# microsoft/MaskFlownet

Hardware: AMD Instinct MI355X
Metric: image-pairs/s MaskFlownet-S 384x512 fwd hot path (correlation + deformable conv + warp) (higher is better)
Workload: dtype f32

## Files before the change

include/mfn_hip.h:

```cpp
#ifndef MFN_HIP_H
#define MFN_HIP_H

#include <stddef.h>

#ifdef __cplusplus
extern "C" {
#endif

#define MFN_ABI_VERSION 1

#define MFN_OK 0
#define MFN_E_NULL (-1)
#define MFN_E_SHAPE (-2)
#define MFN_E_PARAM (-3)
#define MFN_E_UNSUPPORTED (-4)
#define MFN_E_WORKSPACE (-5)
#define MFN_E_ALIGN (-6)

#define MFN_REQ_NULL 0
#define MFN_REQ_WRITE 1
#define MFN_REQ_ADD 3

int mfn_abi_version(void);
const char *mfn_version_string(void);
// ... 196 lines not shown
int mfn_graph_destroy(void *graph_exec);

int mfn_profile_enable(int on);
int mfn_profile_reset(void);
int mfn_profile_tag(const char *tag);
int mfn_profile_query(const char *name_substr, int *launches, double *total_ms);
int mfn_profile_dump(char *buf, int cap);

#define MFN_ARITH_DEFAULT (-1)
#define MFN_ARITH_FP32 0
#define MFN_ARITH_BF16X3 1
int mfn_set_arithmetic(const char *op, int mode);
int mfn_get_arithmetic(const char *op, int *mode);

int mfn_debug_set_timeline(void *device_buffer);
int mfn_set_tuning(const char *key, int value);
int mfn_get_tuning(const char *key, int *value);

#ifdef __cplusplus
}
#endif
#endif
```

maskflownet_amd/_abi.py:

```python
import ctypes as C
from types import SimpleNamespace

_f = C.c_void_p
_i = C.c_int
_s = C.c_void_p
_pi = C.POINTER(C.c_int)

SIGNATURES = {
    "last_error": (C.c_char_p, []),
    "correlation_out_shape": (_i, [_i] * 7 + [_pi, _pi, _pi]),
    "correlation_fwd": (_i, [_f, _f, _f] + [_i] * 10 + [_s]),
    "correlation_workspace_bytes": (C.c_size_t, [_i] * 10),
    "correlation_fwd_ws": (_i, [_f, _f, _f] + [_i] * 10 + [C.c_void_p, C.c_size_t, _s]),
    "correlation_fwd_act": (_i, [_f, _f, _f] + [_i] * 11 + [C.c_void_p, C.c_size_t, _s]),
    "correlation_fwd_into": (_i, [_f, _f, _f, C.c_longlong] + [_i] * 11 + [C.c_void_p, C.c_size_t, _s]),
    "warp_fwd": (_i, [_f, _f, _f] + [_i] * 5 + [_s]),
    "grid_generator_warp": (_i, [_f, _f, _i, _i, _i, _s]),
    "grid_generator_affine": (_i, [_f, _f, _i, _i, _i, _s]),
    "bilinear_sampler_fwd": (_i, [_f, _f, _f] + [_i] * 6 + [_s]),
    "bilinear_sampler_bwd": (_i, [_f] * 5 + [_i] * 8 + [_s]),
    "grid_generator_warp_bwd": (_i, [_f, _f] + [_i] * 4 + [_s]),
    "deform_conv_out_shape": (_i, [_i] * 10 + [_pi, _pi]),
    "deform_conv_workspace_bytes": (C.c_size_t, [_i] * 15),
    "deform_conv_fwd": (_i, [_f] * 5 + [_i] * 15 + [C.c_void_p, C.c_size_t, _s]),
    "deform_conv_shared_fwd": (_i, [_f, _f, C.c_float, C.c_float, _f, _f, _f] + [_i] * 12 + [C.c_void_p, C.c_size_t, _s]),
    "offsets_from_flow": (_i, [_f, _f, _i, _i, _i, _i, C.c_float, C.c_float, _s]),
    "offsets_from_flow_bwd": (_i, [_f, _f, _i, _i, _i, _i, C.c_float, C.c_float, _i, _s]),
    "deform_conv_shared_bwd_workspace_bytes": (C.c_size_t, [_i] * 12),
    "deform_conv_shared_bwd": (_i, [_f, _f, _f, C.c_float, C.c_float, _f, _f, _f, _f, _f] + [_i] * 16 + [C.c_void_p, C.c_size_t, _s]),
    "debug_set_timeline": (_i, [C.c_void_p]),
    "correlation_bwd": (_i, [_f] * 5 + [_i] * 12 + [_s]),
    "warp_bwd": (_i, [_f] * 5 + [_i] * 7 + [_s]),
    "deform_conv_packed_weight_bytes": (C.c_size_t, [_i] * 15),
    "deform_conv_pack_weights": (_i, [_f] + [_i] * 15 + [C.c_void_p, C.c_size_t, C.POINTER(C.c_ulonglong), _s]),
    "deform_conv_fwd_packed": (_i, [_f, _f, C.c_void_p, C.c_size_t, C.c_ulonglong, _f, _f] + [_i] * 15 + [C.c_void_p, C.c_size_t, _s]),
    "deform_conv_shared_fwd_packed": (_i, [_f, _f, C.c_float, C.c_float, C.c_void_p, C.c_size_t, C.c_ulonglong, _f, _f] + [_i] * 12 + [C.c_void_p, C.c_size_t, _s]),
    "upsample_fwd": (_i, [_f, _f] + [_i] * 5 + [_s]),
    "deform_conv_matching_fwd": (_i, [_f, _f, C.c_float, C.c_float, _f, C.c_void_p, C.c_size_t, C.c_ulonglong, _f, _f, _f, _i, _f]
                                 + [_i] * 12 + [C.c_void_p, C.c_size_t, _s]),
    "deform_conv_bwd_workspace_bytes": (C.c_size_t, [_i] * 15),
    "deform_conv_bwd": (_i, [_f] * 8 + [_i] * 19 + [C.c_void_p, C.c_size_t, _s]),
    "conv2d_out_shape": (_i, [_i] * 13 + [_pi, _pi]),
    "conv2d_workspace_bytes": (C.c_size_t, [_i] * 15),
    "conv2d_packed_weight_bytes": (C.c_size_t, [_i] * 15),
    "conv2d_pack_weights": (_i, [_f] + [_i] * 15 + [C.c_void_p, C.c_size_t, C.POINTER(C.c_ulonglong), _s]),
# ... 75 lines not shown
```

maskflownet_amd/csrc/api_impl.inc:

```

#include <atomic>
#include <math.h>
#include <stdarg.h>
#include <stdio.h>
#include <string.h>

#include "kernels/correlation.h"
#include "kernels/correlation_direct.h"
#include "kernels/correlation_gram.h"
#include "kernels/correlation_gramk.h"
#include "kernels/conv_wgrad.h"
#include "kernels/deform_conv.h"
#include "kernels/deform_conv_mma.h"
#include "kernels/warp.h"
#include "kernels/upsample.h"
#include "kernels/predict.h"
#include "kernels/augment.h"
#include "kernels/loss.h"
#include "kernels/optimizer.h"
#include "kernels/batch.h"
#include "kernels/ingest.h"
#include "kernels/backward.h"
#include "kernels/dc_backward.h"
#include "kernels/conv.h"
// ... 9 lines not shown
  vsnprintf(g_err, sizeof(g_err), fmt, ap);
  va_end(ap);
  return code;
}
static int hipfail(int rc, const char *what) {
  if (rc == 0) return 0;
  snprintf(g_err, sizeof(g_err), "%s: HIP error %d (%s)", what, rc, hipGetErrorString((hipError_t)rc));
  return rc;
}
static inline bool aligned(const void *p, size_t a) { return ((uintptr_t)p % a) == 0; }

Tuning g_tuning;
struct Arith { std::atomic<int> corr{-1}, deform{-1}, conv{-1}; };
static Arith t_arith;
void *g_timeline = nullptr;
struct Settings { Tuning t; int corr, deform, conv; };
static Settings settings_now() { return Settings{g_tuning, t_arith.corr.load(), t_arith.deform.load(), t_arith.conv.load()}; }

static int corr_shape(int H, int W, int md, int kernel, int s1, int s2, int pad, int *tc, int *th, int *tw) {
  if (H <= 0 || W <= 0) return fail(MFN_E_SHAPE, "correlation: H=%d W=%d must be positive", H, W);
  if (md < 0 || kernel < 1 || s1 < 1 || s2 < 1 || pad < 0)
    return fail(MFN_E_PARAM, "correlation: bad parameter (max_displacement=%d kernel_size=%d stride1=%d stride2=%d pad_size=%d)",
                md, kernel, s1, s2, pad);
  if ((kernel % 2) == 0) return fail(MFN_E_PARAM, "correlation: kernel size should be odd number (got %d)", kernel);
  const int Hp = H + 2 * pad, Wp = W + 2 * pad;
  const int border = md + (kernel - 1) / 2;
  const int th_ = (int)ceilf((float)(Hp - border * 2) / (float)s1);
  const int tw_ = (int)ceilf((float)(Wp - border * 2) / (float)s1);
  if (th_ < 1 || tw_ < 1)
    return fail(MFN_E_SHAPE, "correlation: Correlation cannot be done with current settings. Neighborhood and kernel don't fit in blob");
// ... 286 lines not shown
  if (H + 2 * ph < dh * (kh - 1) + 1 || W + 2 * pw < dw * (kw - 1) + 1 || ho < 1 || wo < 1)
    return fail(MFN_E_SHAPE, "deform_conv: kernel size exceed input");
  if (Ho) *Ho = ho;
  if (Wo) *Wo = wo;
  return 0;
}

static bool dc_mfma_ok(const Settings &st, int kh, int kw, int groups, int dg) {
  return (st.t.path_generic & 2) == 0 && kh == 3 && kw == 3 && groups == 1 && dg == 1;
}

struct DcPlan {
  int mt, pt, nw, ksb, mgroups, ncp_pad, cps_per_slice;
  int mma;
  int kw, ring, groups, gps;
  int tile_w, tiles_x, tiles_y, ntiles;
  size_t wt_bytes, partial_bytes, mg_words;
};
#ifndef MFN_DCM_CONFIGS
#define MFN_DCM_CONFIGS(X) X(1, 4, 1) X(2, 3, 4) X(2, 2, 2) X(3, 1, 6) X(1, 1, 8) X(1, 1, 4) X(1, 1, 2) X(1, 1, 1)
#endif
static bool dcm_config_ok(int mt, int pt, int kw) {
#define X(a, b, c) if (mt == a && pt == b && kw == c) return true;
  MFN_DCM_CONFIGS(X)
#undef X
  return false;
}
static DcPlan dc_plan(const Settings &st, int Cin, int Cout, int N, int Ho, int Wo, bool mma_shape) {
  DcPlan pl;
  memset(&pl, 0, sizeof(pl));
  const long P = (long)N * Ho * Wo;
  const int mtiles = (Cout + 31) / 32;
  int mt = 1;
  pl.tile_w = Wo >= 8 ? 8 : 0;
  if (pl.tile_w) {
    pl.tiles_x = (Wo + pl.tile_w - 1) / pl.tile_w;
// ... 9 lines not shown
    pl.groups = Cin / 16;
    pl.ring = 3;
    int cmt = 1, cpt = 1, ckw = pl.groups % 8 == 0 ? 8 : (pl.groups % 4 == 0 ? 4 : (pl.groups % 2 == 0 ? 2 : 1));
    if (mtiles == 1 && tiles >= 1024) { cpt = 4; ckw = 1; }
    else if (mtiles == 2 && tiles >= 384 && pl.groups % 4 == 0) {
      cmt = 2; cpt = 3; ckw = 4;
      if ((tiles + 2) / 3 > 256 && (tiles + 1) / 2 <= 512) { cpt = 2; ckw = 2; }
    }
    else if (mtiles == 3 && pl.groups % 6 == 0) { cmt = 3; ckw = 6; }
    else if (tiles >= 1024) { cpt = 4; ckw = 1; }
    if (st.t.dc_mt > 0 && st.t.dc_pt > 0 && st.t.dc_nw > 0) {
      cmt = st.t.dc_mt; cpt = st.t.dc_pt; ckw = st.t.dc_nw / (cpt > 0 ? cpt : 1);
    }
    if (!dcm_config_ok(cmt, cpt, ckw) || pl.groups % ckw != 0 || cmt > mtiles) { cmt = 1; cpt = 1; ckw = 1; }
    pl.mt = cmt; pl.pt = cpt; pl.kw = ckw; pl.nw = cpt * ckw; pl.ksb = 1;
    pl.mgroups = (mtiles + cmt - 1) / cmt;
    pl.gps = pl.groups / ckw;
    pl.mg_words = (size_t)(pl.groups * 9 + dcm_kc(cmt, ckw)) * (3 * cmt * 256);
    pl.wt_bytes = (pl.mgroups * pl.mg_words * sizeof(float) + 255) / 256 * 256;
    pl.partial_bytes = 0;
    return pl;
  }
  pl.mt = mt;
  pl.mma = 0;
  pl.mgroups = (mtiles + mt - 1) / mt;
  const int ncp = (Cin + 1) / 2;
  int pt = st.t.dc_pt;
  if (!(pt == 1 || pt == 2 || pt == 4)) {
    double best = 1e30;
    pt = 1;
// ... 147 lines not shown
  p.cps_per_slice = pl.cps_per_slice;
  p.ksb = pl.ksb;
  p.mgroups = pl.mgroups;
  p.tile_w = pl.tile_w; p.tiles_x = pl.tiles_x; p.tiles_y = pl.tiles_y; p.ntiles = pl.ntiles;
  p.inv_tpi = pl.tile_w ? 1.0f / (float)(pl.tiles_y * pl.tiles_x) : 0.f;
  p.inv_tiles_x = pl.tile_w ? 1.0f / (float)pl.tiles_x : 0.f;
  p.partial = pl.ksb > 1 ? (float *)partial_base : nullptr;
  rc = -1000;
  if (pl.mma == 2) {
    if (!aligned(p.x, 16) || !aligned(p.out, 16) || !aligned(p.wt, 16))
      return fail(MFN_E_ALIGN, "%s: x, out and the packed weights must be 16-byte aligned for the matrix-core layout these weights were packed in "
                  "(pass the raw weights, or pack under mfn_set_arithmetic(\"deformable_convolution\", MFN_ARITH_FP32))", what);
    p.dcm_groups = pl.groups;
    p.dcm_gps = pl.gps;
    p.xcd = pl.mgroups == 1 || cdiv(pl.ntiles, pl.pt) % 8 == 0;
#define X(a, b, c) else if (pl.mt == a && pl.pt == b && pl.kw == c) rc = dc_mma_launch<a, b, c, 3>(p, s);
    if (false) {}
    MFN_DCM_CONFIGS(X)
#undef X
    if (rc == -1000) return fail(MFN_E_UNSUPPORTED, "%s: no matrix-core kernel for mt=%d pt=%d kw=%d", what, pl.mt, pl.pt, pl.kw);
    return hipfail(rc, what);
  }
  if (pl.nw == 8) rc = dc_lds_launch<1, 1, 8>(p, s, "dc_lds");
  else if (pl.pt == 1) rc = dc_lds_launch<1, 1>(p, s, "dc_lds");
  else if (pl.pt == 2) rc = dc_lds_launch<1, 2>(p, s, "dc_lds");
  else if (pl.pt == 4) rc = dc_lds_launch<1, 4>(p, s, "dc_lds");
  if (rc == -1000) return fail(MFN_E_UNSUPPORTED, "%s: no kernel for mt=%d pt=%d", what, pl.mt, pl.pt);
  if (rc) return hipfail(rc, what);
  if (pl.ksb > 1) {
    DcReduceParams rp{p.partial, p.bias, p.out, (size_t)p.Cout * p.P, pl.ksb, p.Cout, (size_t)p.Ho * p.Wo,
                      p.ep_mask, p.ep_add, p.ep_leaky};
    rc = dc_reduce_launch(rp, s);
// ... 1511 lines not shown
int MFN_API(set_arithmetic)(const char *op, int mode) {
  if (mode < -1 || mode > 1) return fail(MFN_E_PARAM, "set_arithmetic: mode %d is none of MFN_ARITH_DEFAULT / _FP32 / _BF16X3", mode);
  if (op && !strcmp(op, "all")) { t_arith.corr = mode; t_arith.deform = mode; t_arith.conv = mode; return 0; }
  std::atomic<int> *slot = arith_slot(op);
  if (!slot) return fail(MFN_E_PARAM, "set_arithmetic: unknown operator '%s'", op ? op : "(null)");
  *slot = mode;
  return 0;
}
int MFN_API(get_arithmetic)(const char *op, int *mode) {
  std::atomic<int> *slot = arith_slot(op);
  if (!slot || !mode) return fail(MFN_E_PARAM, "get_arithmetic: unknown operator '%s'", op ? op : "(null)");
  *mode = *slot;
  return 0;
}

int MFN_API(set_tuning)(const char *key, int value) {
  int *slot = key ? g_tuning.slot(key) : nullptr;
  if (!slot) return fail(MFN_E_PARAM, "set_tuning: unknown key '%s'", key ? key : "(null)");
  *slot = value;
  return 0;
}
int MFN_API(get_tuning)(const char *key, int *value) {
  int *slot = key ? g_tuning.slot(key) : nullptr;
  if (!slot || !value) return fail(MFN_E_PARAM, "get_tuning: unknown key '%s'", key ? key : "(null)");
  *value = *slot;
  return 0;
}

}
```

maskflownet_amd/csrc/kernels/deform_conv_mma.h:

```cpp
#pragma once
#include "deform_conv.h"
#include "msplit.h"

namespace mfn {

constexpr int DCM_XW_F = 512;
template <bool BIG, int RING> struct DcmWin {
  static constexpr int ROWS = BIG ? 16 : 12, COLS = BIG ? 24 : 20, C4 = COLS / 4, CH = ROWS * COLS;
  static constexpr int CHS = BIG ? CH : 268;
  static constexpr bool IS_BIG = BIG;
  static constexpr int NI = BIG ? 3 : 2, SLOT_F = BIG ? 768 : 512;
  static constexpr int DEPTH = BIG ? (RING * DCM_XW_F) / 768 : RING;
  static_assert(CHS % 4 == 0 && CHS >= CH && CHS + CH <= SLOT_F && CHS + CH <= NI * 256 && DEPTH >= 2, "the pair's window fits its slot and its transfers");
};

template <int RING> struct DcmWinConv {
  static constexpr int ROWS = 6, COLS = 16, C4 = 4, CH = ROWS * COLS, CHS = 104;
  static constexpr int NI = 1, SLOT_F = 256;
  static constexpr int DEPTH = (RING * DCM_XW_F) / SLOT_F;
  static_assert(CHS % 4 == 0 && CHS >= CH && CHS + CH <= SLOT_F && DEPTH >= 2, "the pair's window fits one transfer");
};

constexpr int dcm_kc(int mt, int kw) { return mt * kw == 1 ? 3 : 1; }
constexpr int dcm_nstage(int mt, int pt, int kw, int ring) {
// ... 5 lines not shown
constexpr int dcm_min_waves(int mt, int nw) {
  const int fit = (nw + 3) / 4, want = mt == 1 ? 3 : (mt == 2 ? 2 : 1);
  return fit > want ? fit : want;
}

#ifndef MFN_DCM_ABLATE
#define MFN_DCM_ABLATE 0
#endif
#ifndef MFN_DCM_MSPLIT
#define MFN_DCM_MSPLIT (MT <= 2)
#endif
#ifndef MFN_DCM_MINW
#define MFN_DCM_MINW(mt, nw) dcm_min_waves(mt, nw)
#endif

template <int MT, int PT, int KW, int RING> struct DcmGeom {
  static constexpr int NW = PT * KW, NTH = NW * 64;
  static constexpr int KC = dcm_kc(MT, KW);
  static constexpr int NSTAGE = dcm_nstage(MT, PT, KW, RING);
  static constexpr int STEP_W = 3 * MT * 256;
  static constexpr int WI_TOTAL = KW * KC * 3 * MT;
  static constexpr int NI = (WI_TOTAL + NW - 1) / NW;
  static constexpr int NI_MIN = WI_TOTAL / NW;
  static constexpr int STAGE_W = WI_TOTAL * 256;
  static constexpr int XW_OFF = NSTAGE * STAGE_W;
  static constexpr int T8_OFF = XW_OFF + NW * RING * DCM_XW_F;
  static constexpr int DUMP_OFF = T8_OFF + NW * 512;
  static constexpr int LDS_W = DUMP_OFF + 256;
  static_assert(LDS_W * 4 <= 160 * 1024, "a block's LDS must fit the CU");
  static constexpr int RED_TS = 40, RED_TILE = 32 * RED_TS;
  static constexpr int RED_W = KW > 1 ? PT * KW * MT * RED_TILE : 0;
  static_assert(RED_W <= DUMP_OFF, "every slice's partial tiles fit the block's LDS at once");
  static constexpr int RED_ROWS = 32 * MT, RED_SLAB = RED_ROWS / KW, RED_PASSES = (RED_SLAB + 7) / 8;
  static_assert(RED_ROWS % KW == 0, "the K slices divide the tile's filter rows evenly (every shipped tiling; an uneven split needs a clipped last slab)");
};

template <int KC, int NSTAGE, int RING, int NI, int XW_NI, int REQ = 0> constexpr int dcm_wait_count(int s) {
  int issued = 0, result = 1000;
  int stampW[64] = {}, stampX[80] = {};
  for (int u = 0; u < 45; ++u) {
    const int ss = u % 9, grp = u / 9;
    if (u == 36 + s) {
      int need = -1;
      if (ss % KC == 0 && stampW[u / KC] > need) need = stampW[u / KC];
      if (ss != 7) {
        const int np = ss == 8 ? 8 * (grp + 1) : 8 * grp + ss + 1;
        if (stampX[np] > need) need = stampX[np];
      }
      result = need < 0 ? 1000 : issued - need;
    }
    if (ss % KC == 0) { issued += NI; stampW[u / KC + NSTAGE - 1] = issued; }
    if (ss < 8) { issued += XW_NI; stampX[8 * grp + ss + RING] = issued; }
    if (ss != 7) issued += REQ;
  }
  return result;
}
template <int KC, int NSTAGE, int RING, int NI, int XW_NI, int REQ> constexpr int dcm_landed_count(int s) {
  int issued = 0, last_req = 0, result = 0;
  for (int u = 0; u < 45; ++u) {
    const int ss = u % 9;
    if (ss % KC == 0) issued += NI;
    if (ss < 8) issued += XW_NI;
    if (ss != 7) {
      issued += REQ;
      if (u == 36 + s) result = issued - last_req;
      last_req = issued;
    }
  }
  return result;
}

template <int KC, int NSTAGE, int RING, int NI, int XW_NI> constexpr unsigned dcm_wait_mask(int s) {
  const int v = dcm_wait_count<KC, NSTAGE, RING, NI, XW_NI>(s);
  unsigned m = 0;
  for (int q = 0; q < 9; ++q) {
    if (dcm_wait_count<KC, NSTAGE, RING, NI, XW_NI>(q) != v) continue;
// ... 24 lines not shown
  }
  mfn_bf16x8 h, mm, l;
  mfn_split3x8(x, h, mm, l);
  float *base = p.wt + (size_t)mg * p.mg_words + ((size_t)grp * 9 + s) * (3 * p.MT * 256) + (size_t)(kb * 32 + m) * 4;
  mfn_write_bf16x8(base + (0 * p.MT + ft) * 256, h);
  mfn_write_bf16x8(base + (1 * p.MT + ft) * 256, mm);
  mfn_write_bf16x8(base + (2 * p.MT + ft) * 256, l);
}
inline int dcm_pack_launch(DcmPackParams pp, hipStream_t stream) {
  const size_t total = (size_t)pp.mgroups * pp.ngroups * 9 * pp.MT * 64;
  return launch("dcm_pack_weights", dcm_pack_weights_kernel, dim3((unsigned)((total + 255) / 256)), dim3(256), 0, stream, pp);
}

struct DcmB { mfn_bf16x8 h, m, l; };

template <int MT, int PT, int KW, int RING, bool CONV = false>
__global__ __launch_bounds__(PT * KW * 64, MFN_DCM_MINW(MT, PT * KW)) void dc_mma_kernel(DeformParams p) {
  using G = DcmGeom<MT, PT, KW, RING>;
  constexpr int NW = G::NW, KC = G::KC, NI = G::NI, NIW = G::NI_MIN;
  constexpr int NACC = MT == 1 ? 2 : 1;
  constexpr bool PRIVATE_W = PT == 1;
  static_assert(!PRIVATE_W || G::NI * NW == G::WI_TOTAL, "one pixel tile: the slices' blocks divide evenly over the waves");
  static_assert(9 % KC == 0, "chunk boundaries at fixed steps of a group");
  static_assert(RING >= 3 && RING * DCM_XW_F >= 32 * 40, "the epilogue transposes a tile through the wave's window ring");
  MFN_DYN_SHARED(float, lds);

  const int tid = threadIdx.x;
  const int lane = tid & 63;
  const int wave = MFN_UNIFORM(tid >> 6);
  const int kb = lane >> 5, j = lane & 31;
  const int pt = wave / KW, kw = wave % KW;
  MFN_STAMP(p.timeline, 0);
  const int bx = p.xcd ? (int)mfn_xcd_remap(blockIdx.x, gridDim.x) : (int)blockIdx.x;
  const int tile = bx * PT + pt;
// ... 4 lines not shown
  const size_t xns = p.x_nstride ? p.x_nstride : (size_t)p.Cin * plane;

  const int gps = p.dcm_gps;
  const size_t mg_words = (size_t)(p.dcm_groups * 9 + KC) * G::STEP_W;
  const mfn_rsrc_t wrsrc = mfn_make_rsrc(p.wt + (size_t)mg * mg_words, (unsigned)(mg_words * 4));
  unsigned voffW[NI];
  MFN_UNROLL
  for (int i = 0; i < NI; ++i) {
    const int ii = PRIVATE_W ? wave * (KC * 3 * MT) + i : i * NW + wave;
    const int k = ii / (KC * 3 * MT), rem = ii - k * (KC * 3 * MT);
    voffW[i] = ii < G::WI_TOTAL ? (unsigned)((((size_t)k * gps * 9) * G::STEP_W + (size_t)rem * 256) * 4) + (unsigned)lane * 16u : 0xFFFFFF00u;
  }
  auto issue_w = [&](int ch) {
    float *buf = lds + (ch % G::NSTAGE) * G::STAGE_W;
    const unsigned soff = ch * KC < gps * 9 ? (unsigned)((size_t)ch * KC * G::STEP_W * 4) : 0x7FFFFF00u;
    if (MFN_DCM_ABLATE & 32) return;
    MFN_UNROLL
    for (int i = 0; i < NI; ++i) {
      const int ii = PRIVATE_W ? wave * (KC * 3 * MT) + i : i * NW + wave;
      if (ii < G::WI_TOTAL) mfn_dma16_so(wrsrc, buf + ii * 256, voffW[i], soff);
    }
  };

  MFN_UNROLL
  for (int ch = 0; ch < G::NSTAGE - 1; ++ch) issue_w(ch);

  int n, ty, tx;
  {
    auto divmod = [](int a, int b, float inv_b, int &q, int &r) {
      q = (int)((float)a * inv_b);
      r = a - q * b;
      if (r < 0) { --q; r += b; }
      if (r >= b) { ++q; r -= b; }
    };
    const int tl = min(tile, p.ntiles - 1);
    int rt;
    divmod(tl, p.tiles_y * p.tiles_x, p.inv_tpi, n, rt);
    divmod(rt, p.tiles_x, p.inv_tiles_x, ty, tx);
  }
  const int tile_ho0 = ty * 4, tile_wo0 = tx * 8;
// ... 256 lines not shown
    }
  };
  DcmB B;
  GramSel sel;
  if (MFN_DCM_MSPLIT) sel = gram_make_sel(lane);
  mfn_bf16x8 ah[MT], am[MT], al[MT];
  auto a_read = [&](const float *a) {
    MFN_UNROLL
    for (int ft = 0; ft < MT; ++ft) {
      if (MFN_DCM_ABLATE & 64) { ah[ft] = am[ft] = al[ft] = B.h; continue; }
      al[ft] = mfn_read_bf16x8(a + (2 * MT + ft) * 256);
      ah[ft] = mfn_read_bf16x8(a + (0 * MT + ft) * 256);
      am[ft] = mfn_read_bf16x8(a + (1 * MT + ft) * 256);
    }
  };
  auto mma_issue = [&](const DcmB &b) {
    if (MFN_DCM_ABLATE & 1) {
      MFN_UNROLL
      for (int ft = 0; ft < MT; ++ft) acc[ft][0][0] += mfn_bf16_at(reinterpret_cast<const float *>(&ah[ft]), 0) + mfn_bf16_at(reinterpret_cast<const float *>(&al[ft]), 1) + mfn_bf16_at(reinterpret_cast<const float *>(&am[ft]), 2) + mfn_bf16_at(reinterpret_cast<const float *>(&b.l), 0);
      return;
    }
#define MFN_DCM_(A_, B_, P_)                                                                      \
  MFN_UNROLL                                                                                      \
  for (int ft = 0; ft < MT; ++ft) acc[ft][(P_) % NACC] = MFN_MFMA_32x32x16_BF16(A_[ft], B_, acc[ft][(P_) % NACC]);
    MFN_DCM_(al, b.h, 0)
    MFN_DCM_(ah, b.l, 1)
    MFN_DCM_(am, b.m, 0)
    MFN_DCM_(am, b.h, 1)
    MFN_DCM_(ah, b.m, 0)
    MFN_DCM_(ah, b.h, 1)
// ... 20 lines not shown
        MFN_UNROLL
        for (int ft = 0; ft < MT; ++ft) {
          const float wv = mfn_bf16_at(a + (0 * MT + ft) * 256, t) + mfn_bf16_at(a + (1 * MT + ft) * 256, t) + mfn_bf16_at(a + (2 * MT + ft) * 256, t);
          acc[ft][0] = MFN_MFMA_32x32x2(wv, cvt, acc[ft][0]);
        }
      } else {
        *t8dst = cvt;
      }
    }
  };

  float *xt8 = lds + G::T8_OFF + wave * 512 + lane;
  auto first_operand = [&](auto win_c, auto out_c) {
    using WN = decltype(win_c);
    MFN_WAIT_VM(0);
    float x8[8] = {0.f, 0.f, 0.f, 0.f, 0.f, 0.f, 0.f, 0.f}, c8 = 0.f;
    if (fast) {
      if (decltype(out_c)::value) lanes_request(0, std::integral_constant<int, 1>{});
      cols_gather(0, win_c);
      if (decltype(out_c)::value) {
        lanes_landed(std::integral_constant<int, 1>{}, std::integral_constant<int, 0>{});
        lanes_request(1, std::integral_constant<int, 0>{});
      }
      cols_finish(x8, c8);
    }
    xt8[0] = c8;
    if (MFN_DCM_MSPLIT) gram_msplit8(x8, sel, B.h, B.m, B.l);
    else mfn_split3x8(x8, B.h, B.m, B.l);
    MFN_STAMP2(p.timeline, 4);
  };

  auto run_groups = [&](auto win_c, auto out_c) {
    using WN = decltype(win_c);
    constexpr int CPG = 9 / KC;
    if (decltype(out_c)::value) lanes_setup();
    first_operand(win_c, out_c);
    MFN_NOUNROLL
    for (int g = 0; g < gps; ++g) {
      mfn_static_for<9>([&](auto s_c) {
        constexpr int S = decltype(s_c)::value;
        constexpr bool OUT = decltype(out_c)::value;
        constexpr int NWAIT = dcm_wait_count<KC, G::NSTAGE, WN::DEPTH, NIW, WN::NI, OUT ? 16 : 0>(S);
        if (NWAIT < 1000) MFN_WAIT_VM(NWAIT < 63 ? NWAIT : 63);
        const int ch = g * CPG + S / KC;
        constexpr int kk = S % KC;
        const int kn = S == 8 ? (g + 1) * 8 : g * 8 + S + 1;
        constexpr int E = S == 8 ? 7 : S;
        if (kk == 0) {
          MFN_WAIT_LGKM0();
          if (!PRIVATE_W && !(MFN_DCM_ABLATE & 128)) MFN_RAW_BARRIER();
          if (S == 0 && g == 0) MFN_STAMP(p.timeline, 1);
          issue_w(ch + G::NSTAGE - 1);
        }
        if (S < 8) issue_x(g * 8 + S + WN::DEPTH, win_c);
        if (OUT && S != 7) lanes_request(S == 8 ? g * 8 + 9 : g * 8 + S + 2, std::integral_constant<int, (E + 1) & 1>{});
        const float *a = lds + (ch % G::NSTAGE) * G::STAGE_W + (size_t)(kw * KC + kk) * G::STEP_W + (kb * 32 + j) * 4;
        float x8[8];
        a_read(a);
        if (S != 7) cols_gather(kn, win_c);
        mma_issue(B);
        if (OUT && S != 7)
          lanes_landed(std::integral_constant<int, E & 1>{},
                       std::integral_constant<int, dcm_landed_count<KC, G::NSTAGE, WN::DEPTH, NIW, WN::NI, 16>(S)>{});
        if (S == 7) {
          MFN_UNROLL
          for (int e = 0; e < 8; ++e) x8[e] = xt8[e * 64];
        } else {
          float c8;
          cols_finish(x8, c8);
          xt8[(S == 8 ? 0 : S + 1) * 64] = c8;
        }
#ifdef MFN_DCM_SPLIT_PACKED
        if (!(MFN_DCM_ABLATE & 8)) mfn_split3x8(x8, B.h, B.m, B.l);
#else
        if (!(MFN_DCM_ABLATE & 8)) {
          if (MFN_DCM_MSPLIT) gram_msplit8(x8, sel, B.h, B.m, B.l);
          else mfn_split3x8_scalar(x8, B.h, B.m, B.l);
        }
#endif
        MFN_SCHED_BARRIER();
      });
    }
  };
  auto run_pertap = [&]() {
    using WN = DcmWin<false, RING>;
    first_operand(WN{}, std::false_type{});
    const int nsteps = gps * 9;
    int s = 0, kl = 0;
    MFN_NOUNROLL
    for (int t = 0; t < nsteps; ++t) {
      mfn_static_for<9>([&](auto s_c) {
        constexpr int S = decltype(s_c)::value;
        constexpr int NWAIT = dcm_wait_count<KC, G::NSTAGE, WN::DEPTH, NIW, WN::NI>(S);
        constexpr unsigned MASK = dcm_wait_mask<KC, G::NSTAGE, WN::DEPTH, NIW, WN::NI>(S);
        if (NWAIT < 1000 && MASK != 0 && ((MASK >> s) & 1u)) MFN_WAIT_VM(NWAIT < 63 ? NWAIT : 63);
      });
      const int ch = t / KC, kk = t - ch * KC;
      if (kk == 0) {
        MFN_WAIT_LGKM0();
        if (!PRIVATE_W) MFN_RAW_BARRIER();
        if (t == 0) MFN_STAMP(p.timeline, 1);
        issue_w(ch + G::NSTAGE - 1);
      }
      if (s < 8) issue_x(kl + WN::DEPTH, WN{});
      const float *a = lds + (ch % G::NSTAGE) * G::STAGE_W + (size_t)(kw * KC + kk) * G::STEP_W + (kb * 32 + j) * 4;
      if (s < 8) pertap_pair(kl, a, xt8 + (kl & 7) * 64);
      else { a_read(a); mma_issue(B); }
      if (s == 7) {
        float x8[8];
        MFN_UNROLL
        for (int e = 0; e < 8; ++e) x8[e] = xt8[e * 64];
        mfn_split3x8(x8, B.h, B.m, B.l);
      }
      if (s < 8) ++kl;
      s = s == 8 ? 0 : s + 1;
    }
  };
  if constexpr (CONV) run_groups(DcmWinConv<RING>{}, std::false_type{});
  else {
    if (!fast) run_pertap();
// ... 115 lines not shown
      MFN_WAIT_LGKM0();
      MFN_UNROLL
      for (int r = 0; r < 16; ++r) tr[((r & 3) + 8 * (r >> 2) + 4 * kb) * TS + j] = fin[mt][r];
      MFN_WAIT_LGKM0();
      MFN_UNROLL
      for (int i = 0; i < 4; ++i) {
        const int ol = i * 8 + orow;
        const float4 v = *reinterpret_cast<const float4 *>(tr + ol * TS + px0);
        finish_row(m0 + mt * 32 + ol, v, bq[i], addv[i], true);
      }
    }
  }
  MFN_STAMP(p.timeline, 3);
}

template <int MT, int PT, int KW, int RING, bool CONV = false>
inline int dc_mma_launch(const DeformParams &p, hipStream_t stream, const char *name = "dc_mma") {
  using G = DcmGeom<MT, PT, KW, RING>;
  const int bx = cdiv(p.ntiles, PT);
  if (bx <= 0) return 0;
  return launch(name, dc_mma_kernel<MT, PT, KW, RING, CONV>, dim3(bx, 1, p.mgroups), dim3(G::NTH), (size_t)G::LDS_W * sizeof(float), stream, p);
}
inline bool dcm_conv_shape_ok(int N, size_t x_nstride, int H, int W, int kh, int kw, int sh, int sw, int ph, int pw, int dh, int dw, int groups) {
  return kh == 3 && kw == 3 && sh == 1 && sw == 1 && ph == 1 && pw == 1 && dh == 1 && dw == 1 && groups == 1 && W % 4 == 0 && W >= 8 &&
         H >= 1 && (size_t)N * x_nstride < ((size_t)1 << 30);
}

inline bool dcm_shape_ok(int N, int Cin, int H, int W, int Ho, int Wo, int kh, int kw, int sh, int sw, int ph, int pw, int dh, int dw,
                         int groups, int dg) {
  return kh == 3 && kw == 3 && sh == 1 && sw == 1 && ph == 1 && pw == 1 && dh == 1 && dw == 1 && groups == 1 && dg == 1 && Ho == H &&
         Wo == W && W % 4 == 0 && W >= 8 && H >= 1 && Cin % 16 == 0 && (size_t)N * Cin * H * W < ((size_t)1 << 30);
}

}
```

maskflownet_amd/csrc/mfn_rt.h:

```cpp
#pragma once

#if defined(MFN_EMU)
#include "hipemu.h"
typedef f32x16_emu f32x16;
typedef f32x4_emu f32x4;
struct f4u { float x, y, z, w; };
static inline f4u mfn_load4u(const float *p) { f4u v; memcpy(&v, p, 16); return v; }
struct f3u { float x, y, z; };
static inline f3u mfn_load3u(const float *p) { f3u v; memcpy(&v, p, 12); return v; }
static inline int mfn_f2i(float f) { int i; memcpy(&i, &f, 4); return i; }
struct f2u { float x, y; };
static inline f2u mfn_load2u(const float *p) { f2u v; memcpy(&v, p, 8); return v; }
struct f32x2 { float x, y; };
static inline f32x2 mfn_f2(float x, float y) { return f32x2{x, y}; }
static inline f32x2 mfn_fma2(f32x2 a, f32x2 b, f32x2 c) { return f32x2{fmaf(a.x, b.x, c.x), fmaf(a.y, b.y, c.y)}; }
template <bool HI> static inline void mfn_pk_fma_swbc(f32x2 &acc, f32x2 a, f32x2 b) {
  const float bb = HI ? b.y : b.x;
  acc = f32x2{fmaf(a.y, bb, acc.x), fmaf(a.x, bb, acc.y)};
}
static inline void mfn_fmac_inorder(float &acc, float a, float b) { acc = fmaf(a, b, acc); }
struct f32x4v { float x, y, z, w; };
static inline f32x4v mfn_lds_read4(const float *p) { return f32x4v{p[0], p[1], p[2], p[3]}; }
static inline f32x2 mfn_lo2(f32x4v v) { return f32x2{v.x, v.y}; }
static inline f32x2 mfn_hi2(f32x4v v) { return f32x2{v.z, v.w}; }
// ... 109 lines not shown
  else memset(dst, 0, 16);
}
static inline void mfn_gload4_async(f32x4_emu &dst, const float *base_uniform, unsigned byteoff) {
  memcpy(&dst, (const char *)base_uniform + byteoff, 16);
}
static inline void mfn_bload1x4_async(float &d0, float &d1, float &d2, float &d3, mfn_rsrc_t r, unsigned voff, unsigned soff,
                                      unsigned long long lanes) {
  if (!((lanes >> hipemu::t_lane) & 1ull)) return;
  float *d[4] = {&d0, &d1, &d2, &d3};
  for (int k = 0; k < 4; ++k) {
    const unsigned off = voff + 4u * k;
    if ((unsigned long long)off + soff + 4 <= r.nrec) memcpy(d[k], r.base + off + soff, 4);
    else *d[k] = 0.f;
  }
}
#define MFN_LANDED4(a, b, c, d, n) ((void)0)
#define MFN_REGFENCE4(a, b, c, d) ((void)0)
#define MFN_REGFENCE9(v) ((void)0)
#define MFN_REGFENCE8(a, b, c, d, e, f, g, h) ((void)0)
#define MFN_SCHED_GROUP(mask, n) ((void)0)
#define MFN_WAIT_VM(n) (hipemu::wave().bar.arrive_and_wait())
#define MFN_WAIT_LGKM0() (hipemu::wave().bar.arrive_and_wait())
static inline void mfn_wait_vm_dyn(unsigned) { hipemu::wave().bar.arrive_and_wait(); }
#define MFN_RAW_BARRIER() __syncthreads()
#define MFN_LDS_BARRIER() __syncthreads()
#define MFN_COMPILER_FENCE() ((void)0)
#define MFN_STAMP(buf, k) ((void)0)
#define MFN_STAMP2(buf, k) ((void)0)
#define MFN_STAMP_INFO(buf, val) ((void)0)
#define MFN_CYCLES() 0ull
// ... 291 lines not shown
  const unsigned long long sb = ((unsigned long long)hi << 32) | lo;
  asm volatile("s_nop 4\n\tglobal_load_dwordx4 %0, %1, %2" : "=v"(dst) : "v"(byteoff), "s"(sb) : "memory");
}
__device__ __forceinline__ void mfn_bload1x4_async(float &d0, float &d1, float &d2, float &d3, mfn_rsrc_t rsrc, unsigned voff, unsigned soff,
                                                   unsigned long long lanes) {
  const unsigned so = __builtin_amdgcn_readfirstlane(soff);
  unsigned long long saved;
  asm volatile("s_and_saveexec_b64 %4, %8\n\ts_nop 4\n\t"
               "buffer_load_dword %0, %5, %6, %7 offen\n\tbuffer_load_dword %1, %5, %6, %7 offen offset:4\n\t"
               "buffer_load_dword %2, %5, %6, %7 offen offset:8\n\tbuffer_load_dword %3, %5, %6, %7 offen offset:12\n\t"
               "s_mov_b64 exec, %4"
               : "=&v"(d0), "=&v"(d1), "=&v"(d2), "=&v"(d3), "=&s"(saved) : "v"(voff), "s"(rsrc), "s"(so), "s"(lanes) : "memory", "scc");
}
#define MFN_LANDED4(a, b, c, d, n) asm volatile("s_waitcnt vmcnt(%4)" : "+v"(a), "+v"(b), "+v"(c), "+v"(d) : "n"(n) : "memory")
#define MFN_REGFENCE4(a, b, c, d) asm volatile("" : "+v"(a), "+v"(b), "+v"(c), "+v"(d) : : "memory")
#define MFN_REGFENCE9(v) asm volatile("" : "+v"((v)[0]), "+v"((v)[1]), "+v"((v)[2]), "+v"((v)[3]), "+v"((v)[4]), "+v"((v)[5]), "+v"((v)[6]), "+v"((v)[7]), "+v"((v)[8]))
#define MFN_REGFENCE8(a, b, c, d, e, f, g, h) asm volatile("" : "+v"(a), "+v"(b), "+v"(c), "+v"(d), "+v"(e), "+v"(f), "+v"(g), "+v"(h))
#define MFN_RAW_BARRIER() __builtin_amdgcn_s_barrier()
#define MFN_COMPILER_FENCE() asm volatile("" ::: "memory")
#define MFN_LDS_BARRIER() asm volatile("s_waitcnt lgkmcnt(0)\n\ts_barrier" ::: "memory")
#define MFN_CYCLES() ((unsigned long long)clock64())
#ifndef MFN_TIMELINE
#define MFN_TIMELINE 0
#endif
#if !MFN_TIMELINE
#define MFN_STAMP(buf, k) ((void)0)
#define MFN_STAMP2(buf, k) ((void)0)
#define MFN_STAMP_INFO(buf, val) ((void)0)
#else
#define MFN_STAMP_INFO(buf, val)                                                                            \
// ... 112 lines not shown
```

Baseline: 60660.

## Stream deformable-conv filter operands straight into registers instead of LDS staging

Adds an AREG variant of the matrix-core deformable conv kernel. Each wave loads its packed bf16 filter tiles directly from global memory into double-buffered registers one tap ahead, instead of staging them through a multi-stage LDS ring. This removes the LDS writes and reads for weights, along with the per-chunk LDS waits and block barriers. The wait-count bookkeeping is extended to cover the new register loads. In exchange it uses more VGPRs and issues more global loads per wave, since weights are no longer shared across waves through LDS. It is enabled by default for three tile configs and also adds a debug query that reports the chosen plan.

```diff
diff --git a/include/mfn_hip.h b/include/mfn_hip.h
--- a/include/mfn_hip.h
+++ b/include/mfn_hip.h
@@ -234,6 +234,7 @@
 int mfn_get_arithmetic(const char *op, int *mode);
 
 int mfn_debug_set_timeline(void *device_buffer);
+int mfn_debug_last_dc_plan(int *mt, int *pt, int *kw, int *areg);
 int mfn_set_tuning(const char *key, int value);
 int mfn_get_tuning(const char *key, int *value);
 
diff --git a/maskflownet_amd/_abi.py b/maskflownet_amd/_abi.py
--- a/maskflownet_amd/_abi.py
+++ b/maskflownet_amd/_abi.py
@@ -29,6 +29,7 @@
     "deform_conv_shared_bwd_workspace_bytes": (C.c_size_t, [_i] * 12),
     "deform_conv_shared_bwd": (_i, [_f, _f, _f, C.c_float, C.c_float, _f, _f, _f, _f, _f] + [_i] * 16 + [C.c_void_p, C.c_size_t, _s]),
     "debug_set_timeline": (_i, [C.c_void_p]),
+    "debug_last_dc_plan": (_i, [_pi, _pi, _pi, _pi]),
     "correlation_bwd": (_i, [_f] * 5 + [_i] * 12 + [_s]),
     "warp_bwd": (_i, [_f] * 5 + [_i] * 7 + [_s]),
     "deform_conv_packed_weight_bytes": (C.c_size_t, [_i] * 15),
diff --git a/maskflownet_amd/csrc/api_impl.inc b/maskflownet_amd/csrc/api_impl.inc
--- a/maskflownet_amd/csrc/api_impl.inc
+++ b/maskflownet_amd/csrc/api_impl.inc
@@ -47,6 +47,7 @@
 struct Arith { std::atomic<int> corr{-1}, deform{-1}, conv{-1}; };
 static Arith t_arith;
 void *g_timeline = nullptr;
+static thread_local int t_last_dc_plan[4] = {0, 0, 0, 0};
 struct Settings { Tuning t; int corr, deform, conv; };
 static Settings settings_now() { return Settings{g_tuning, t_arith.corr.load(), t_arith.deform.load(), t_arith.conv.load()}; }
 
@@ -363,12 +364,22 @@
   int mt, pt, nw, ksb, mgroups, ncp_pad, cps_per_slice;
   int mma;
   int kw, ring, groups, gps;
+  int areg;
   int tile_w, tiles_x, tiles_y, ntiles;
   size_t wt_bytes, partial_bytes, mg_words;
 };
 #ifndef MFN_DCM_CONFIGS
 #define MFN_DCM_CONFIGS(X) X(1, 4, 1) X(2, 3, 4) X(2, 2, 2) X(3, 1, 6) X(1, 1, 8) X(1, 1, 4) X(1, 1, 2) X(1, 1, 1)
 #endif
+#ifndef MFN_DCM_AREG_CONFIGS
+#define MFN_DCM_AREG_CONFIGS(X) X(1, 4, 1) X(3, 1, 6) X(1, 1, 8)
+#endif
+static bool dcm_areg_config_ok(int mt, int pt, int kw) {
+#define X(a, b, c) if (mt == a && pt == b && kw == c) return true;
+  MFN_DCM_AREG_CONFIGS(X)
+#undef X
+  return false;
+}
 static bool dcm_config_ok(int mt, int pt, int kw) {
 #define X(a, b, c) if (mt == a && pt == b && kw == c) return true;
   MFN_DCM_CONFIGS(X)
@@ -408,6 +419,7 @@
     }
     if (!dcm_config_ok(cmt, cpt, ckw) || pl.groups % ckw != 0 || cmt > mtiles) { cmt = 1; cpt = 1; ckw = 1; }
     pl.mt = cmt; pl.pt = cpt; pl.kw = ckw; pl.nw = cpt * ckw; pl.ksb = 1;
+    pl.areg = dcm_areg_config_ok(cmt, cpt, ckw) && !(st.t.dc_off & 4);
     pl.mgroups = (mtiles + cmt - 1) / cmt;
     pl.gps = pl.groups / ckw;
     pl.mg_words = (size_t)(pl.groups * 9 + dcm_kc(cmt, ckw)) * (3 * cmt * 256);
@@ -585,8 +597,12 @@
     p.dcm_groups = pl.groups;
     p.dcm_gps = pl.gps;
     p.xcd = pl.mgroups == 1 || cdiv(pl.ntiles, pl.pt) % 8 == 0;
+    t_last_dc_plan[0] = pl.mt; t_last_dc_plan[1] = pl.pt; t_last_dc_plan[2] = pl.kw; t_last_dc_plan[3] = pl.areg;
+#define X(a, b, c) else if (pl.areg && pl.mt == a && pl.pt == b && pl.kw == c) rc = dc_mma_launch<a, b, c, 3, false, true>(p, s);
+    if (false) {}
+    MFN_DCM_AREG_CONFIGS(X)
+#undef X
 #define X(a, b, c) else if (pl.mt == a && pl.pt == b && pl.kw == c) rc = dc_mma_launch<a, b, c, 3>(p, s);
-    if (false) {}
     MFN_DCM_CONFIGS(X)
 #undef X
     if (rc == -1000) return fail(MFN_E_UNSUPPORTED, "%s: no matrix-core kernel for mt=%d pt=%d kw=%d", what, pl.mt, pl.pt, pl.kw);
@@ -2128,6 +2144,14 @@
   return 0;
 }
 
+int MFN_API(debug_last_dc_plan)(int *mt, int *pt, int *kw, int *areg) {
+  if (mt) *mt = t_last_dc_plan[0];
+  if (pt) *pt = t_last_dc_plan[1];
+  if (kw) *kw = t_last_dc_plan[2];
+  if (areg) *areg = t_last_dc_plan[3];
+  return 0;
+}
+
 int MFN_API(set_tuning)(const char *key, int value) {
   int *slot = key ? g_tuning.slot(key) : nullptr;
   if (!slot) return fail(MFN_E_PARAM, "set_tuning: unknown key '%s'", key ? key : "(null)");
diff --git a/maskflownet_amd/csrc/kernels/deform_conv_mma.h b/maskflownet_amd/csrc/kernels/deform_conv_mma.h
--- a/maskflownet_amd/csrc/kernels/deform_conv_mma.h
+++ b/maskflownet_amd/csrc/kernels/deform_conv_mma.h
@@ -43,7 +43,7 @@
 #define MFN_DCM_MINW(mt, nw) dcm_min_waves(mt, nw)
 #endif
 
-template <int MT, int PT, int KW, int RING> struct DcmGeom {
+template <int MT, int PT, int KW, int RING, bool AREG = false> struct DcmGeom {
   static constexpr int NW = PT * KW, NTH = NW * 64;
   static constexpr int KC = dcm_kc(MT, KW);
   static constexpr int NSTAGE = dcm_nstage(MT, PT, KW, RING);
@@ -52,43 +52,45 @@
   static constexpr int NI = (WI_TOTAL + NW - 1) / NW;
   static constexpr int NI_MIN = WI_TOTAL / NW;
   static constexpr int STAGE_W = WI_TOTAL * 256;
-  static constexpr int XW_OFF = NSTAGE * STAGE_W;
+  static constexpr int XW_OFF = AREG ? 0 : NSTAGE * STAGE_W;
   static constexpr int T8_OFF = XW_OFF + NW * RING * DCM_XW_F;
-  static constexpr int DUMP_OFF = T8_OFF + NW * 512;
-  static constexpr int LDS_W = DUMP_OFF + 256;
-  static_assert(LDS_W * 4 <= 160 * 1024, "a block's LDS must fit the CU");
   static constexpr int RED_TS = 40, RED_TILE = 32 * RED_TS;
   static constexpr int RED_W = KW > 1 ? PT * KW * MT * RED_TILE : 0;
-  static_assert(RED_W <= DUMP_OFF, "every slice's partial tiles fit the block's LDS at once");
+  static constexpr int LDS_W = NSTAGE * STAGE_W + NW * RING * DCM_XW_F + NW * 512 + 256;
+  static_assert(LDS_W * 4 <= 160 * 1024, "a block's LDS must fit the CU");
+  static_assert(RED_W <= LDS_W - 256, "every slice's partial tiles fit the block's LDS at once");
   static constexpr int RED_ROWS = 32 * MT, RED_SLAB = RED_ROWS / KW, RED_PASSES = (RED_SLAB + 7) / 8;
   static_assert(RED_ROWS % KW == 0, "the K slices divide the tile's filter rows evenly (every shipped tiling; an uneven split needs a clipped last slab)");
 };
 
-template <int KC, int NSTAGE, int RING, int NI, int XW_NI, int REQ = 0> constexpr int dcm_wait_count(int s) {
+template <int KC, int NSTAGE, int RING, int NI, int XW_NI, int REQ = 0, int AR = 0> constexpr int dcm_wait_count(int s) {
   int issued = 0, result = 1000;
-  int stampW[64] = {}, stampX[80] = {};
+  int stampW[64] = {}, stampX[80] = {}, stampA[48] = {};
   for (int u = 0; u < 45; ++u) {
     const int ss = u % 9, grp = u / 9;
     if (u == 36 + s) {
       int need = -1;
-      if (ss % KC == 0 && stampW[u / KC] > need) need = stampW[u / KC];
+      if (NI > 0 && ss % KC == 0 && stampW[u / KC] > need) need = stampW[u / KC];
+      if (AR > 0 && ss != 0 && stampA[u] > need) need = stampA[u];
       if (ss != 7) {
         const int np = ss == 8 ? 8 * (grp + 1) : 8 * grp + ss + 1;
         if (stampX[np] > need) need = stampX[np];
       }
       result = need < 0 ? 1000 : issued - need;
     }
-    if (ss % KC == 0) { issued += NI; stampW[u / KC + NSTAGE - 1] = issued; }
+    if (NI > 0 && ss % KC == 0) { issued += NI; stampW[u / KC + NSTAGE - 1] = issued; }
+    if (AR > 0) { issued += AR; stampA[u + 1] = issued; }
     if (ss < 8) { issued += XW_NI; stampX[8 * grp + ss + RING] = issued; }
     if (ss != 7) issued += REQ;
   }
   return result;
 }
-template <int KC, int NSTAGE, int RING, int NI, int XW_NI, int REQ> constexpr int dcm_landed_count(int s) {
+template <int KC, int NSTAGE, int RING, int NI, int XW_NI, int REQ, int AR = 0> constexpr int dcm_landed_count(int s) {
   int issued = 0, last_req = 0, result = 0;
   for (int u = 0; u < 45; ++u) {
     const int ss = u % 9;
-    if (ss % KC == 0) issued += NI;
+    if (NI > 0 && ss % KC == 0) issued += NI;
+    issued += AR;
     if (ss < 8) issued += XW_NI;
     if (ss != 7) {
       issued += REQ;
@@ -143,10 +145,12 @@
 
 struct DcmB { mfn_bf16x8 h, m, l; };
 
-template <int MT, int PT, int KW, int RING, bool CONV = false>
+template <int MT, int PT, int KW, int RING, bool CONV = false, bool AREG = false>
 __global__ __launch_bounds__(PT * KW * 64, MFN_DCM_MINW(MT, PT * KW)) void dc_mma_kernel(DeformParams p) {
-  using G = DcmGeom<MT, PT, KW, RING>;
-  constexpr int NW = G::NW, KC = G::KC, NI = G::NI, NIW = G::NI_MIN;
+  static_assert(!(CONV && AREG), "the plain-convolution form keeps the LDS path");
+  using G = DcmGeom<MT, PT, KW, RING, AREG>;
+  constexpr int NW = G::NW, KC = G::KC, NI = G::NI, NIW = AREG ? 0 : G::NI_MIN;
+  constexpr int AR = AREG ? 3 * MT : 0;
   constexpr int NACC = MT == 1 ? 2 : 1;
   constexpr bool PRIVATE_W = PT == 1;
   static_assert(!PRIVATE_W || G::NI * NW == G::WI_TOTAL, "one pixel tile: the slices' blocks divide evenly over the waves");
@@ -181,16 +185,24 @@
   auto issue_w = [&](int ch) {
     float *buf = lds + (ch % G::NSTAGE) * G::STAGE_W;
     const unsigned soff = ch * KC < gps * 9 ? (unsigned)((size_t)ch * KC * G::STEP_W * 4) : 0x7FFFFF00u;
-    if (MFN_DCM_ABLATE & 32) return;
+    if (AREG || (MFN_DCM_ABLATE & 32)) return;
     MFN_UNROLL
     for (int i = 0; i < NI; ++i) {
       const int ii = PRIVATE_W ? wave * (KC * 3 * MT) + i : i * NW + wave;
       if (ii < G::WI_TOTAL) mfn_dma16_so(wrsrc, buf + ii * 256, voffW[i], soff);
     }
   };
-
-  MFN_UNROLL
-  for (int ch = 0; ch < G::NSTAGE - 1; ++ch) issue_w(ch);
+  f32x4 A[2][3 * MT];
+  const unsigned voffA = (unsigned)(((size_t)(wave % KW) * gps * 9) * G::STEP_W * 4) + (unsigned)lane * 16u;
+  auto request_a = [&](int st, auto set_c) {
+    mfn_bload4_blocks_async(A[decltype(set_c)::value], wrsrc, voffA, (unsigned)((size_t)st * G::STEP_W * 4), st < gps * 9);
+  };
+
+  if constexpr (AREG) request_a(0, std::integral_constant<int, 0>{});
+  else {
+    MFN_UNROLL
+    for (int ch = 0; ch < G::NSTAGE - 1; ++ch) issue_w(ch);
+  }
 
   int n, ty, tx;
   {
@@ -477,6 +489,15 @@
       am[ft] = mfn_read_bf16x8(a + (1 * MT + ft) * 256);
     }
   };
+  auto a_from = [&](auto set_c) {
+    constexpr int SET = decltype(set_c)::value;
+    MFN_UNROLL
+    for (int ft = 0; ft < MT; ++ft) {
+      ah[ft] = mfn_bf16x8_of(A[SET][0 * MT + ft]);
+      am[ft] = mfn_bf16x8_of(A[SET][1 * MT + ft]);
+      al[ft] = mfn_bf16x8_of(A[SET][2 * MT + ft]);
+    }
+  };
   auto mma_issue = [&](const DcmB &b) {
     if (MFN_DCM_ABLATE & 1) {
       MFN_UNROLL
@@ -527,6 +548,7 @@
   auto first_operand = [&](auto win_c, auto out_c) {
     using WN = decltype(win_c);
     MFN_WAIT_VM(0);
+    if constexpr (AREG) mfn_landed_blocks<0>(A[0]);
     float x8[8] = {0.f, 0.f, 0.f, 0.f, 0.f, 0.f, 0.f, 0.f}, c8 = 0.f;
     if (fast) {
       if (decltype(out_c)::value) lanes_request(0, std::integral_constant<int, 1>{});
@@ -553,13 +575,17 @@
       mfn_static_for<9>([&](auto s_c) {
         constexpr int S = decltype(s_c)::value;
         constexpr bool OUT = decltype(out_c)::value;
-        constexpr int NWAIT = dcm_wait_count<KC, G::NSTAGE, WN::DEPTH, NIW, WN::NI, OUT ? 16 : 0>(S);
-        if (NWAIT < 1000) MFN_WAIT_VM(NWAIT < 63 ? NWAIT : 63);
+        constexpr int NWAIT = dcm_wait_count<KC, G::NSTAGE, WN::DEPTH, NIW, WN::NI, OUT ? 16 : 0, AR>(S);
+        if constexpr (AREG && S != 0) mfn_landed_blocks<(NWAIT < 63 ? NWAIT : 63)>(A[S & 1]);
+        else if (NWAIT < 1000) MFN_WAIT_VM(NWAIT < 63 ? NWAIT : 63);
         const int ch = g * CPG + S / KC;
         constexpr int kk = S % KC;
         const int kn = S == 8 ? (g + 1) * 8 : g * 8 + S + 1;
         constexpr int E = S == 8 ? 7 : S;
-        if (kk == 0) {
+        if constexpr (AREG) {
+          if (S == 0 && g == 0) MFN_STAMP(p.timeline, 1);
+          request_a(g * 9 + S + 1, std::integral_constant<int, (S + 1) & 1>{});
+        } else if (kk == 0) {
           MFN_WAIT_LGKM0();
           if (!PRIVATE_W && !(MFN_DCM_ABLATE & 128)) MFN_RAW_BARRIER();
           if (S == 0 && g == 0) MFN_STAMP(p.timeline, 1);
@@ -569,12 +595,13 @@
         if (OUT && S != 7) lanes_request(S == 8 ? g * 8 + 9 : g * 8 + S + 2, std::integral_constant<int, (E + 1) & 1>{});
         const float *a = lds + (ch % G::NSTAGE) * G::STAGE_W + (size_t)(kw * KC + kk) * G::STEP_W + (kb * 32 + j) * 4;
         float x8[8];
-        a_read(a);
+        if constexpr (AREG) a_from(std::integral_constant<int, S & 1>{});
+        else a_read(a);
         if (S != 7) cols_gather(kn, win_c);
         mma_issue(B);
         if (OUT && S != 7)
           lanes_landed(std::integral_constant<int, E & 1>{},
-                       std::integral_constant<int, dcm_landed_count<KC, G::NSTAGE, WN::DEPTH, NIW, WN::NI, 16>(S)>{});
+                       std::integral_constant<int, dcm_landed_count<KC, G::NSTAGE, WN::DEPTH, NIW, WN::NI, 16, AR>(S)>{});
         if (S == 7) {
           MFN_UNROLL
           for (int e = 0; e < 8; ++e) x8[e] = xt8[e * 64];
@@ -591,6 +618,11 @@
           else mfn_split3x8_scalar(x8, B.h, B.m, B.l);
         }
 #endif
+        if constexpr (AREG && S == 8) {
+          mfn_landed_blocks<(OUT ? 16 : 0)>(A[1]);
+          MFN_UNROLL
+          for (int b = 0; b < 3 * MT; ++b) A[0][b] = A[1][b];
+        }
         MFN_SCHED_BARRIER();
       });
     }
@@ -609,14 +641,17 @@
         if (NWAIT < 1000 && MASK != 0 && ((MASK >> s) & 1u)) MFN_WAIT_VM(NWAIT < 63 ? NWAIT : 63);
       });
       const int ch = t / KC, kk = t - ch * KC;
-      if (kk == 0) {
+      if (AREG) {
+        if (t == 0) MFN_STAMP(p.timeline, 1);
+      } else if (kk == 0) {
         MFN_WAIT_LGKM0();
         if (!PRIVATE_W) MFN_RAW_BARRIER();
         if (t == 0) MFN_STAMP(p.timeline, 1);
         issue_w(ch + G::NSTAGE - 1);
       }
       if (s < 8) issue_x(kl + WN::DEPTH, WN{});
-      const float *a = lds + (ch % G::NSTAGE) * G::STAGE_W + (size_t)(kw * KC + kk) * G::STEP_W + (kb * 32 + j) * 4;
+      const float *a = AREG ? p.wt + (size_t)mg * mg_words + ((size_t)kw * gps * 9 + t) * G::STEP_W + (kb * 32 + j) * 4
+                            : lds + (ch % G::NSTAGE) * G::STAGE_W + (size_t)(kw * KC + kk) * G::STEP_W + (kb * 32 + j) * 4;
       if (s < 8) pertap_pair(kl, a, xt8 + (kl & 7) * 64);
       else { a_read(a); mma_issue(B); }
       if (s == 7) {
@@ -762,12 +797,12 @@
   MFN_STAMP(p.timeline, 3);
 }
 
-template <int MT, int PT, int KW, int RING, bool CONV = false>
+template <int MT, int PT, int KW, int RING, bool CONV = false, bool AREG = false>
 inline int dc_mma_launch(const DeformParams &p, hipStream_t stream, const char *name = "dc_mma") {
-  using G = DcmGeom<MT, PT, KW, RING>;
+  using G = DcmGeom<MT, PT, KW, RING, AREG>;
   const int bx = cdiv(p.ntiles, PT);
   if (bx <= 0) return 0;
-  return launch(name, dc_mma_kernel<MT, PT, KW, RING, CONV>, dim3(bx, 1, p.mgroups), dim3(G::NTH), (size_t)G::LDS_W * sizeof(float), stream, p);
+  return launch(name, dc_mma_kernel<MT, PT, KW, RING, CONV, AREG>, dim3(bx, 1, p.mgroups), dim3(G::NTH), (size_t)G::LDS_W * sizeof(float), stream, p);
 }
 inline bool dcm_conv_shape_ok(int N, size_t x_nstride, int H, int W, int kh, int kw, int sh, int sw, int ph, int pw, int dh, int dw, int groups) {
   return kh == 3 && kw == 3 && sh == 1 && sw == 1 && ph == 1 && pw == 1 && dh == 1 && dw == 1 && groups == 1 && W % 4 == 0 && W >= 8 &&
diff --git a/maskflownet_amd/csrc/mfn_rt.h b/maskflownet_amd/csrc/mfn_rt.h
--- a/maskflownet_amd/csrc/mfn_rt.h
+++ b/maskflownet_amd/csrc/mfn_rt.h
@@ -147,6 +147,15 @@
     else *d[k] = 0.f;
   }
 }
+template <int NB> static inline void mfn_bload4_blocks_async(f32x4_emu (&d)[NB], mfn_rsrc_t r, unsigned voff, unsigned soff, bool live) {
+  for (int b = 0; b < NB; ++b) {
+    const unsigned long long off = (unsigned long long)voff + soff + 1024u * b;
+    if (live && off + 16 <= r.nrec) memcpy(&d[b], r.base + off, 16);
+    else memset(&d[b], 0, 16);
+  }
+}
+template <int N, int NB> static inline void mfn_landed_blocks(f32x4_emu (&)[NB]) { hipemu::wave().bar.arrive_and_wait(); }
+static inline mfn_bf16x8 mfn_bf16x8_of(const f32x4_emu &q) { mfn_bf16x8 v; memcpy(&v, &q, 16); return v; }
 #define MFN_LANDED4(a, b, c, d, n) ((void)0)
 #define MFN_REGFENCE4(a, b, c, d) ((void)0)
 #define MFN_REGFENCE9(v) ((void)0)
@@ -468,6 +477,41 @@
 }
 #define MFN_LANDED4(a, b, c, d, n) asm volatile("s_waitcnt vmcnt(%4)" : "+v"(a), "+v"(b), "+v"(c), "+v"(d) : "n"(n) : "memory")
 #define MFN_REGFENCE4(a, b, c, d) asm volatile("" : "+v"(a), "+v"(b), "+v"(c), "+v"(d) : : "memory")
+template <int NB>
+__device__ __forceinline__ void mfn_bload4_blocks_async(f32x4 (&d)[NB], mfn_rsrc_t rsrc, unsigned voff, unsigned soff, bool live) {
+  static_assert(NB == 3 || NB == 6 || NB == 9, "one, two or three filter tiles of three terms");
+  const unsigned s0 = __builtin_amdgcn_readfirstlane(live ? soff : 0x7FFFFF00u);
+  const unsigned s1 = __builtin_amdgcn_readfirstlane(live ? soff + 4096u : 0x7FFFFF00u);
+  const unsigned s2 = __builtin_amdgcn_readfirstlane(live ? soff + 8192u : 0x7FFFFF00u);
+  if constexpr (NB == 3) {
+    asm volatile("s_nop 4\n\tbuffer_load_dwordx4 %0, %3, %4, %5 offen\n\tbuffer_load_dwordx4 %1, %3, %4, %5 offen offset:1024\n\t"
+                 "buffer_load_dwordx4 %2, %3, %4, %5 offen offset:2048"
+                 : "=&v"(d[0]), "=&v"(d[1]), "=&v"(d[2]) : "v"(voff), "s"(rsrc), "s"(s0) : "memory");
+  } else if constexpr (NB == 6) {
+    asm volatile("s_nop 4\n\tbuffer_load_dwordx4 %0, %6, %7, %8 offen\n\tbuffer_load_dwordx4 %1, %6, %7, %8 offen offset:1024\n\t"
+                 "buffer_load_dwordx4 %2, %6, %7, %8 offen offset:2048\n\tbuffer_load_dwordx4 %3, %6, %7, %8 offen offset:3072\n\t"
+                 "buffer_load_dwordx4 %4, %6, %7, %9 offen\n\tbuffer_load_dwordx4 %5, %6, %7, %9 offen offset:1024"
+                 : "=&v"(d[0]), "=&v"(d[1]), "=&v"(d[2]), "=&v"(d[3]), "=&v"(d[4]), "=&v"(d[5]) : "v"(voff), "s"(rsrc), "s"(s0), "s"(s1) : "memory");
+  } else {
+    asm volatile("s_nop 4\n\tbuffer_load_dwordx4 %0, %9, %10, %11 offen\n\tbuffer_load_dwordx4 %1, %9, %10, %11 offen offset:1024\n\t"
+                 "buffer_load_dwordx4 %2, %9, %10, %11 offen offset:2048\n\tbuffer_load_dwordx4 %3, %9, %10, %11 offen offset:3072\n\t"
+                 "buffer_load_dwordx4 %4, %9, %10, %12 offen\n\tbuffer_load_dwordx4 %5, %9, %10, %12 offen offset:1024\n\t"
+                 "buffer_load_dwordx4 %6, %9, %10, %12 offen offset:2048\n\tbuffer_load_dwordx4 %7, %9, %10, %12 offen offset:3072\n\t"
+                 "buffer_load_dwordx4 %8, %9, %10, %13 offen"
+                 : "=&v"(d[0]), "=&v"(d[1]), "=&v"(d[2]), "=&v"(d[3]), "=&v"(d[4]), "=&v"(d[5]), "=&v"(d[6]), "=&v"(d[7]), "=&v"(d[8])
+                 : "v"(voff), "s"(rsrc), "s"(s0), "s"(s1), "s"(s2) : "memory");
+  }
+}
+template <int N, int NB> __device__ __forceinline__ void mfn_landed_blocks(f32x4 (&d)[NB]) {
+  static_assert(NB == 3 || NB == 6 || NB == 9, "as mfn_bload4_blocks_async");
+  if constexpr (NB == 3) asm volatile("s_waitcnt vmcnt(%3)" : "+v"(d[0]), "+v"(d[1]), "+v"(d[2]) : "n"(N) : "memory");
+  else if constexpr (NB == 6)
+    asm volatile("s_waitcnt vmcnt(%6)" : "+v"(d[0]), "+v"(d[1]), "+v"(d[2]), "+v"(d[3]), "+v"(d[4]), "+v"(d[5]) : "n"(N) : "memory");
+  else
+    asm volatile("s_waitcnt vmcnt(%9)" : "+v"(d[0]), "+v"(d[1]), "+v"(d[2]), "+v"(d[3]), "+v"(d[4]), "+v"(d[5]), "+v"(d[6]), "+v"(d[7]), "+v"(d[8])
+                 : "n"(N) : "memory");
+}
+__device__ __forceinline__ mfn_bf16x8 mfn_bf16x8_of(const f32x4 &q) { return __builtin_bit_cast(mfn_bf16x8, q); }
 #define MFN_REGFENCE9(v) asm volatile("" : "+v"((v)[0]), "+v"((v)[1]), "+v"((v)[2]), "+v"((v)[3]), "+v"((v)[4]), "+v"((v)[5]), "+v"((v)[6]), "+v"((v)[7]), "+v"((v)[8]))
 #define MFN_REGFENCE8(a, b, c, d, e, f, g, h) asm volatile("" : "+v"(a), "+v"(b), "+v"(c), "+v"(d), "+v"(e), "+v"(f), "+v"(g), "+v"(h))
 #define MFN_RAW_BARRIER() __builtin_amdgcn_s_barrier()
```

Measured after the change: 62260 (median of 6 runs). 1.03x the previous value.
